# gargatik/Seamless-Through-Breaking-Rethinking-Image-Stitching-for-Optimal-Alignment

Measured on AMD Instinct MI355X. Metric: stitched image-pairs/s at 512x512, higher is better.
Workload: dtype f32 (decoder contractions, PatchEmbed's third conv and the C = 128 block tails: exact 3xbf16 split of both operands, 6 products on the bf16 matrix cores, fp32 accumulate -- error vs fp64 0.83x the fp32 MFMA chain's; everything else fp32)

## Files before the change

seamless-through-breaking-rethinking-image-stitching-for-optimal-alignment_amd/csrc/mlp_split3.h:

```cpp
#define MS3_W1_B 24576
#define MS3_W2_B 24576
#define MS3_BIAS_B 1024
#define MS3_STAGE_B (MS3_W1_B + MS3_W2_B + MS3_BIAS_B)
#define MS3_PIECES (MS3_STAGE_B / 1024)

typedef unsigned u32x4 __attribute__((ext_vector_type(4)));
typedef __bf16 bf16x2_t __attribute__((ext_vector_type(2)));
typedef float f32x2_t __attribute__((ext_vector_type(2)));

__device__ __forceinline__ unsigned ms3_pk(float a, float b) {
    const f32x2_t v = {a, b};
    return __builtin_bit_cast(unsigned, __builtin_convertvector(v, bf16x2_t));
}
__device__ __forceinline__ void ms3_split_pair(float x0, float x1, unsigned& h, unsigned& m, unsigned& l) {
    h = ms3_pk(x0, x1);
    const float r0 = x0 - __uint_as_float(h << 16), r1 = x1 - __uint_as_float(h & 0xffff0000u);
    m = ms3_pk(r0, r1);
    l = ms3_pk(r0 - __uint_as_float(m << 16), r1 - __uint_as_float(m & 0xffff0000u));
}

__global__ __launch_bounds__(256) void mlp_split3_pack_kernel(const float* __restrict__ w1, const float* __restrict__ b1, const float* __restrict__ w2,
                                                              const float* __restrict__ wp, const float* __restrict__ bp, int hidden,
                                                              unsigned char* __restrict__ image) {
    const int step = blockIdx.y, npre = wp ? 4 : 0;
    const bool pre = step < npre;
    const int c = pre ? step : step - npre;
    unsigned char* st = image + (size_t)step * MS3_STAGE_B;
    const int b = blockIdx.x, t = threadIdx.x;
    if (b < 2) {
        const int idx = b * 256 + t, r = idx >> 4, sl = idx & 15, ks = sl >> 1, lh = sl & 1;
        const float* W = (pre ? wp : w1) + (size_t)(32 * c + r) * 128;
        bf16x8 h, m, l;
#pragma unroll
        for (int e = 0; e < 8; ++e) {
            __bf16 a0, a1, a2;
            st_split3(W[16 * ks + 8 * (e >> 2) + 4 * lh + (e & 3)], a0, a1, a2);
            h[e] = a0; m[e] = a1; l[e] = a2;
        }
        unsigned char* o = st + r * 256 + ((sl ^ (r & 15)) << 4);
        *reinterpret_cast<bf16x8*>(o) = h;
        *reinterpret_cast<bf16x8*>(o + 8192) = m;
        *reinterpret_cast<bf16x8*>(o + 16384) = l;
    } else if (b < 4) {
        const int idx = (b - 2) * 256 + t, r = idx >> 2, sl = idx & 3, ks = sl >> 1, lh = sl & 1;
        bf16x8 h, m, l;
#pragma unroll
        for (int e = 0; e < 8; ++e) {
            __bf16 a0, a1, a2;
            const float v = pre ? 0.f : w2[(size_t)r * hidden + 32 * c + 16 * ks + 8 * (e >> 2) + 4 * lh + (e & 3)];
            st_split3(v, a0, a1, a2);
            h[e] = a0; m[e] = a1; l[e] = a2;
        }
        unsigned char* o = st + MS3_W1_B + r * 64 + ((sl ^ ((r >> 2) & 3)) << 4);
        *reinterpret_cast<bf16x8*>(o) = h;
        *reinterpret_cast<bf16x8*>(o + 8192) = m;
        *reinterpret_cast<bf16x8*>(o + 16384) = l;
    } else {
        float v = 0.f;
        if (t < 32) v = pre ? (bp ? bp[32 * c + t] : 0.f) : b1[32 * c + t];
        reinterpret_cast<float*>(st + MS3_W1_B + MS3_W2_B)[t] = v;
    }
}

#define MS3_SCHED_MFMA_VALU(NV)                                \
    __builtin_amdgcn_sched_group_barrier(0x008, 1, 0);         \
    __builtin_amdgcn_sched_group_barrier(0x002, NV, 0);

#define MS3_NWAVES 4

__device__ __forceinline__ float ms3_gelu(float x) {
    const float u = fabsf(x) * 0.84932180028801904272f;
    const float t = __builtin_amdgcn_rcpf(fmaf(0.2727374808792225f, u, 1.0f));
    float y = fmaf(0.5307027145f, t, -0.7265760135f);
    y = fmaf(y, t, 0.7107068705f);
    y = fmaf(y, t, -0.142248368f);
    y = fmaf(y, t, 0.127414796f);
    y = (y * t) * __builtin_amdgcn_exp2f(-(u * u));
    return fmaf(-fabsf(x), y, fmaxf(x, 0.f));
}

template <bool PROJ>
__global__ __launch_bounds__(256, 1) void rowmlp128_split3_kernel(const st_mlp_desc d, const unsigned char* __restrict__ image, const unsigned image_bytes) {
    extern __shared__ __attribute__((aligned(1024))) unsigned char sm3[];
    const int tid = threadIdx.x, lane = tid & 63, wave = __builtin_amdgcn_readfirstlane(tid >> 6);
    const int li = lane & 31, lh = lane >> 5;
    const int nblk = (d.M + 31) >> 5;
    const int G = (int)gridDim.x;
    const int blk0 = (int)blockIdx.x * MS3_NWAVES;
    const int rounds = blk0 < nblk ? (nblk - blk0 + G * MS3_NWAVES - 1) / (G * MS3_NWAVES) : 0;
    constexpr int npre = PROJ ? 4 : 0;
    const int nhc = d.hidden >> 5, spr = npre + nhc, total = rounds * spr;
    if (total == 0) return;
    const unsigned lds0 = (unsigned)(size_t)(__attribute__((address_space(3))) unsigned char*)sm3;

    int s_dma = 0, g_dma = 0, q_dma = 0;
    const unsigned vlin = (unsigned)lane << 4;
    const i32x4 rsd = make_rsrc(image, image_bytes);
    auto dma_run4 = [&](unsigned lds, unsigned soff) {
        asm volatile("s_mov_b32 m0, %0\n\ts_nop 0\n\t"
                     "buffer_load_dwordx4 %1, %2, %3 offen lds\n\t"
                     "buffer_load_dwordx4 %1, %2, %3 offen offset:1024 lds\n\t"
                     "buffer_load_dwordx4 %1, %2, %3 offen offset:2048 lds\n\t"
                     "buffer_load_dwordx4 %1, %2, %3 offen offset:3072 lds"
                     : : "s"(lds), "v"(vlin), "s"(rsd), "s"(soff) : "memory");
    };
    auto dma_run2 = [&](unsigned lds, unsigned soff) {
        asm volatile("s_mov_b32 m0, %0\n\ts_nop 0\n\t"
                     "buffer_load_dwordx4 %1, %2, %3 offen lds\n\t"
                     "buffer_load_dwordx4 %1, %2, %3 offen offset:1024 lds"
                     : : "s"(lds), "v"(vlin), "s"(rsd), "s"(soff) : "memory");
    };
    auto dma_step = [&]() {
        const unsigned dst = lds0 + (unsigned)(g_dma * MS3_STAGE_B), src = (unsigned)(s_dma * MS3_STAGE_B);
        if (PROJ && s_dma < npre) {
            const unsigned o = (unsigned)wave * 6144u;
            dma_run4(dst + o, src + o);
            dma_run2(dst + o + 4096u, src + o + 4096u);
        } else {
            const unsigned o = (unsigned)wave * 12288u;
            dma_run4(dst + o, src + o);
            dma_run4(dst + o + 4096u, src + o + 4096u);
            dma_run4(dst + o + 8192u, src + o + 8192u);
        }
        if (wave == 0) lds_dma16(rsd, dst + (unsigned)(MS3_W1_B + MS3_W2_B), vlin, src + (unsigned)(MS3_W1_B + MS3_W2_B));
        ++q_dma;
        s_dma = s_dma + 1 == spr ? 0 : s_dma + 1;
        g_dma = g_dma + 1 == 3 ? 0 : g_dma + 1;
    };
    dma_step();
    if (total > 1) dma_step();
    auto step_sync = [&]() {
        asm volatile("s_waitcnt vmcnt(0)" ::: "memory");
        __syncthreads();
        if (q_dma < total) dma_step();
    };

    int fo1[8], fo2[2];
#pragma unroll
    for (int ks = 0; ks < 8; ++ks) fo1[ks] = li * 256 + (((2 * ks + lh) ^ (li & 15)) << 4);
#pragma unroll
    for (int ks = 0; ks < 2; ++ks) fo2[ks] = MS3_W1_B + li * 64 + (((2 * ks + lh) ^ ((li >> 2) & 3)) << 4);

    u32x4 xp[3][8];
    auto split_rows = [&](const float4 (&x)[16]) {
#pragma unroll
        for (int j = 0; j < 16; ++j) {
            unsigned h0, m0, l0, h1, m1, l1;
            ms3_split_pair(x[j].x, x[j].y, h0, m0, l0);
            ms3_split_pair(x[j].z, x[j].w, h1, m1, l1);
            xp[0][j >> 1][2 * (j & 1)] = h0; xp[0][j >> 1][2 * (j & 1) + 1] = h1;
            xp[1][j >> 1][2 * (j & 1)] = m0; xp[1][j >> 1][2 * (j & 1) + 1] = m1;
            xp[2][j >> 1][2 * (j & 1)] = l0; xp[2][j >> 1][2 * (j & 1) + 1] = l1;
        }
    };
#define MS3_BF(v) __builtin_bit_cast(bf16x8, v)
#define MS3_SIX(acc, f, x0, x1, x2)                                                              \
    acc = __builtin_amdgcn_mfma_f32_32x32x16_bf16(MS3_BF(f[2]), MS3_BF(x0), acc, 0, 0, 0);       \
    acc = __builtin_amdgcn_mfma_f32_32x32x16_bf16(MS3_BF(f[0]), MS3_BF(x2), acc, 0, 0, 0);       \
    acc = __builtin_amdgcn_mfma_f32_32x32x16_bf16(MS3_BF(f[1]), MS3_BF(x1), acc, 0, 0, 0);       \
    acc = __builtin_amdgcn_mfma_f32_32x32x16_bf16(MS3_BF(f[1]), MS3_BF(x0), acc, 0, 0, 0);       \
    acc = __builtin_amdgcn_mfma_f32_32x32x16_bf16(MS3_BF(f[0]), MS3_BF(x1), acc, 0, 0, 0);       \
    acc = __builtin_amdgcn_mfma_f32_32x32x16_bf16(MS3_BF(f[0]), MS3_BF(x0), acc, 0, 0, 0);

#define MS3_CHUNK128(acc, g, DMA)                                                                                           \
    {                                                                                                                       \
        const unsigned char* ws_ = sm3 + (g) * MS3_STAGE_B;                                                                 \
        _Pragma("unroll") for (int r = 0; r < 16; ++r) acc[r] = 0.f;                                                        \
        u32x4 f[3], fn[3];                                                                                                  \
        _Pragma("unroll") for (int p = 0; p < 3; ++p) f[p] = *reinterpret_cast<const u32x4*>(ws_ + p * 8192 + fo1[0]);      \
        _Pragma("unroll") for (int ks = 0; ks < 8; ++ks) {                                                                  \
            const int kn = ks + 1 < 8 ? ks + 1 : ks;                                                                        \
            _Pragma("unroll") for (int p = 0; p < 3; ++p) fn[p] = *reinterpret_cast<const u32x4*>(ws_ + p * 8192 + fo1[kn]); \
            MS3_SIX(acc, f, xp[0][ks], xp[1][ks], xp[2][ks])                                                                \
            _Pragma("unroll") for (int p = 0; p < 3; ++p) f[p] = fn[p];                                                     \
            __builtin_amdgcn_sched_barrier(0);                                                                              \
        }                                                                                                                   \
    }
#define MS3_GELU_PAIR(ks, acc, bs)                                                                                          \
    {                                                                                                                       \
        const float2 bq = *reinterpret_cast<const float2*>(bs + 8 * ((2 * (ks)) >> 2) + 4 * lh + ((2 * (ks)) & 3));           \
        unsigned h_, m_, l_;                                                                                                \
        ms3_split_pair(ms3_gelu(acc[2 * (ks)] + bq.x), ms3_gelu(acc[2 * (ks) + 1] + bq.y), h_, m_, l_);                     \
        hp[0][(ks) >> 2][(ks) & 3] = h_; hp[1][(ks) >> 2][(ks) & 3] = m_; hp[2][(ks) >> 2][(ks) & 3] = l_;                  \
    }
#define MS3_PHASE2(wc)                                                                                                      \
    {                                                                                                                       \
        u32x4 f[3], fn[3];                                                                                                  \
        _Pragma("unroll") for (int p = 0; p < 3; ++p) f[p] = *reinterpret_cast<const u32x4*>(wc + p * 8192 + fo2[0]);       \
        _Pragma("unroll") for (int u = 0; u < 8; ++u) {                                                                     \
            const int oc = u >> 1, ks = u & 1, un = u + 1 < 8 ? u + 1 : u;                                                  \
            _Pragma("unroll") for (int p = 0; p < 3; ++p)                                                                   \
                fn[p] = *reinterpret_cast<const u32x4*>(wc + p * 8192 + (un >> 1) * 2048 + fo2[un & 1]);                    \
            MS3_SIX(o[oc], f, hp[0][ks], hp[1][ks], hp[2][ks])                                                              \
            _Pragma("unroll") for (int p = 0; p < 3; ++p) f[p] = fn[p];                                                     \
            __builtin_amdgcn_sched_barrier(0);                                                                              \
        }                                                                                                                   \
    }

    int g = 0;
    auto next_stage = [](int s) { return s + 1 == 3 ? 0 : s + 1; };
    for (int rd = 0; rd < rounds; ++rd) {
        const int blk = blk0 + wave + rd * G * MS3_NWAVES;
        if (blk >= nblk) {
            for (int s = 0; s < spr; ++s) { step_sync(); g = next_stage(g); }
            continue;
        }
        const int row = blk * 32 + li;
        const bool rok = row < d.M;
        const size_t rowc = (size_t)(rok ? row : d.M - 1);
        float4 xf[16];
#pragma unroll
        for (int j = 0; j < 16; ++j) xf[j] = *reinterpret_cast<const float4*>(d.a + rowc * d.lda + 8 * j + 4 * lh);
        if (PROJ) {
            float4 ev[16];
            if (d.res0) {
#pragma unroll
                for (int j = 0; j < 16; ++j) ev[j] = *reinterpret_cast<const float4*>(d.res0 + rowc * d.ld_res0 + 8 * j + 4 * lh);
            } else {
#pragma unroll
                for (int j = 0; j < 16; ++j) ev[j] = make_float4(0.f, 0.f, 0.f, 0.f);
            }
            split_rows(xf);
#pragma unroll
            for (int c = 0; c < 4; ++c) {
                step_sync();
                f32x16 acc;
                MS3_CHUNK128(acc, g, true)
                const float* bs = reinterpret_cast<const float*>(sm3 + g * MS3_STAGE_B + MS3_W1_B + MS3_W2_B);
#pragma unroll
                for (int jj = 0; jj < 4; ++jj) {
                    const float4 bv = *reinterpret_cast<const float4*>(bs + 8 * jj + 4 * lh);
                    const float4 e = ev[4 * c + jj];
                    xf[4 * c + jj] = make_float4((acc[4 * jj] + bv.x) + e.x, (acc[4 * jj + 1] + bv.y) + e.y, (acc[4 * jj + 2] + bv.z) + e.z, (acc[4 * jj + 3] + bv.w) + e.w);
                }
                g = next_stage(g);
            }
        }
        {
            float4 xn[16];
#pragma unroll
            for (int j = 0; j < 16; ++j) xn[j] = xf[j];
            if (d.ln) {
                float s = 0.f;
#pragma unroll
                for (int j = 0; j < 16; ++j) s += (xn[j].x + xn[j].y) + (xn[j].z + xn[j].w);
                s += __shfl_xor(s, 32, 64);
                const float mean = s * (1.0f / 128.0f);
                float v = 0.f;
#pragma unroll
                for (int j = 0; j < 16; ++j) {
                    xn[j].x -= mean; xn[j].y -= mean; xn[j].z -= mean; xn[j].w -= mean;
                    v += (xn[j].x * xn[j].x + xn[j].y * xn[j].y) + (xn[j].z * xn[j].z + xn[j].w * xn[j].w);
                }
                v += __shfl_xor(v, 32, 64);
                const float rstd = 1.0f / sqrtf(v * (1.0f / 128.0f) + d.ln_eps);
#pragma unroll
                for (int j = 0; j < 16; ++j) { xn[j].x *= rstd; xn[j].y *= rstd; xn[j].z *= rstd; xn[j].w *= rstd; }
            }
            split_rows(xn);
        }
        __builtin_amdgcn_sched_barrier(0);
        f32x16 o[4];
#pragma unroll
        for (int oc = 0; oc < 4; ++oc)
#pragma unroll
            for (int r = 0; r < 16; ++r) o[oc][r] = 0.f;
        step_sync();
        f32x16 acc;
        MS3_CHUNK128(acc, g, false)
        u32x4 hp[3][2];
#pragma unroll 1
        for (int hc = 0; hc + 1 < nhc; ++hc) {
            if (hc > 0) step_sync();
            const int gn = next_stage(g);
            const unsigned char* wc = sm3 + g * MS3_STAGE_B;
            const unsigned char* wn = sm3 + gn * MS3_STAGE_B;
            const float* bs = reinterpret_cast<const float*>(wc + MS3_W1_B + MS3_W2_B);
            f32x16 an;
#pragma unroll
            for (int r = 0; r < 16; ++r) an[r] = 0.f;
            {
                u32x4 f[3], fn[3];
#pragma unroll
                for (int p = 0; p < 3; ++p) f[p] = *reinterpret_cast<const u32x4*>(wn + p * 8192 + fo1[0]);
#pragma unroll
                for (int ks = 0; ks < 8; ++ks) {
                    const int kn = ks + 1 < 8 ? ks + 1 : ks;
#pragma unroll
                    for (int p = 0; p < 3; ++p) fn[p] = *reinterpret_cast<const u32x4*>(wn + p * 8192 + fo1[kn]);
                    MS3_SIX(an, f, xp[0][ks], xp[1][ks], xp[2][ks])
                    MS3_GELU_PAIR(ks, acc, bs)
#pragma unroll
                    for (int p = 0; p < 3; ++p) f[p] = fn[p];
                    MS3_SCHED_MFMA_VALU(7) MS3_SCHED_MFMA_VALU(7) MS3_SCHED_MFMA_VALU(7) MS3_SCHED_MFMA_VALU(7) MS3_SCHED_MFMA_VALU(7) MS3_SCHED_MFMA_VALU(7)
                    __builtin_amdgcn_sched_barrier(0);
                }
            }
            MS3_PHASE2(wc)
            acc = an;
            g = gn;
        }
        {
            if (nhc > 1) step_sync();
            const unsigned char* wc = sm3 + g * MS3_STAGE_B;
            const float* bs = reinterpret_cast<const float*>(wc + MS3_W1_B + MS3_W2_B);
#pragma unroll
            for (int ks = 0; ks < 8; ++ks) MS3_GELU_PAIR(ks, acc, bs)
            __builtin_amdgcn_sched_barrier(0);
            MS3_PHASE2(wc)
            g = next_stage(g);
        }
        if (rok) {
            const float* b2p = d.b2;
            asm volatile("" : "+s"(b2p));
#pragma unroll
            for (int oc = 0; oc < 4; ++oc) {
                float4 bb[4], e[4];
#pragma unroll
                for (int jj = 0; jj < 4; ++jj) bb[jj] = *reinterpret_cast<const float4*>(b2p + oc * 32 + 8 * jj + 4 * lh);
                if (d.res) {
#pragma unroll
                    for (int jj = 0; jj < 4; ++jj) e[jj] = *reinterpret_cast<const float4*>(d.res + rowc * d.ld_res + oc * 32 + 8 * jj + 4 * lh);
                } else {
#pragma unroll
                    for (int jj = 0; jj < 4; ++jj) e[jj] = make_float4(0.f, 0.f, 0.f, 0.f);
                }
#pragma unroll
                for (int jj = 0; jj < 4; ++jj) {
                    const int col = oc * 32 + 8 * jj + 4 * lh;
                    const float4 x = xf[4 * oc + jj];
                    float4 v = make_float4((o[oc][4 * jj] + bb[jj].x) + x.x, (o[oc][4 * jj + 1] + bb[jj].y) + x.y, (o[oc][4 * jj + 2] + bb[jj].z) + x.z,
                                           (o[oc][4 * jj + 3] + bb[jj].w) + x.w);
                    if (d.res) { v.x += e[jj].x; v.y += e[jj].y; v.z += e[jj].z; v.w += e[jj].w; }
                    *reinterpret_cast<float4*>(d.out + rowc * d.ldo + col) = v;
                }
            }
        }
    }
}

#define LS3_STAGE_B (MS3_W1_B + MS3_BIAS_B)

__global__ __launch_bounds__(256) void rowlin_split3_pack_kernel(const float* __restrict__ w, const float* __restrict__ b, unsigned char* __restrict__ image) {
    const int c = blockIdx.y, t = threadIdx.x;
    unsigned char* st = image + (size_t)c * LS3_STAGE_B;
    if (blockIdx.x < 2) {
        const int idx = blockIdx.x * 256 + t, r = idx >> 4, sl = idx & 15, ks = sl >> 1, lh = sl & 1;
        const float* W = w + (size_t)(32 * c + r) * 128;
        bf16x8 h, m, l;
#pragma unroll
        for (int e = 0; e < 8; ++e) {
            __bf16 a0, a1, a2;
            st_split3(W[16 * ks + 8 * (e >> 2) + 4 * lh + (e & 3)], a0, a1, a2);
            h[e] = a0; m[e] = a1; l[e] = a2;
        }
        unsigned char* o = st + r * 256 + ((sl ^ (r & 15)) << 4);
        *reinterpret_cast<bf16x8*>(o) = h;
        *reinterpret_cast<bf16x8*>(o + 8192) = m;
        *reinterpret_cast<bf16x8*>(o + 16384) = l;
    } else {
        reinterpret_cast<float*>(st + MS3_W1_B)[t] = (t < 32 && b) ? b[32 * c + t] : 0.f;
    }
}

template <bool AUX>
__global__ __launch_bounds__(256, 2) void rowlin128_split3_kernel(const float* __restrict__ a, const int lda, float* __restrict__ out, const int ldo, const int M,
                                                                  const int N, const int ln, const float ln_eps, const unsigned char* __restrict__ image,
                                                                  const unsigned image_bytes, const float* __restrict__ aux, const int ld_aux, const int row_div) {
    extern __shared__ __attribute__((aligned(1024))) unsigned char sm3[];
    const int tid = threadIdx.x, lane = tid & 63, wave = __builtin_amdgcn_readfirstlane(tid >> 6);
    const int li = lane & 31, lh = lane >> 5;
    const int nblk = (M + 31) >> 5;
    const int G = (int)gridDim.x;
    const int blk0 = (int)blockIdx.x * 4;
    const int rounds = blk0 < nblk ? (nblk - blk0 + G * 4 - 1) / (G * 4) : 0;
    const int spr = N >> 5, total = rounds * spr;
    if (total == 0) return;
    const unsigned lds0 = (unsigned)(size_t)(__attribute__((address_space(3))) unsigned char*)sm3;
    const i32x4 rsd = make_rsrc(image, image_bytes);
    const unsigned vlin = (unsigned)lane << 4;
    int s_dma = 0, g_dma = 0, q_dma = 0;
    auto dma_step = [&]() {
        const unsigned dst = lds0 + (unsigned)(g_dma * LS3_STAGE_B), src = (unsigned)(s_dma * LS3_STAGE_B), o = (unsigned)wave * 6144u;
        asm volatile("s_mov_b32 m0, %0\n\ts_nop 0\n\t"
                     "buffer_load_dwordx4 %1, %2, %3 offen lds\n\t"
                     "buffer_load_dwordx4 %1, %2, %3 offen offset:1024 lds\n\t"
                     "buffer_load_dwordx4 %1, %2, %3 offen offset:2048 lds\n\t"
                     "buffer_load_dwordx4 %1, %2, %3 offen offset:3072 lds"
                     : : "s"(dst + o), "v"(vlin), "s"(rsd), "s"(src + o) : "memory");
        asm volatile("s_mov_b32 m0, %0\n\ts_nop 0\n\t"
                     "buffer_load_dwordx4 %1, %2, %3 offen lds\n\t"
                     "buffer_load_dwordx4 %1, %2, %3 offen offset:1024 lds"
                     : : "s"(dst + o + 4096u), "v"(vlin), "s"(rsd), "s"(src + o + 4096u) : "memory");
        if (wave == 0) lds_dma16(rsd, dst + (unsigned)MS3_W1_B, vlin, src + (unsigned)MS3_W1_B);
        ++q_dma;
        s_dma = s_dma + 1 == spr ? 0 : s_dma + 1;
        g_dma = g_dma + 1 == 3 ? 0 : g_dma + 1;
    };
    dma_step();
    if (total > 1) dma_step();
    int fo1[8];
#pragma unroll
    for (int ks = 0; ks < 8; ++ks) fo1[ks] = li * 256 + (((2 * ks + lh) ^ (li & 15)) << 4);
    int g = 0;
    for (int rd = 0; rd < rounds; ++rd) {
        const int blk = blk0 + wave + rd * G * 4;
        const bool active = blk < nblk;
        const int row = blk * 32 + li;
        const bool rok = active && row < M;
        const size_t rowc = (size_t)(active && row < M ? row : M - 1);
        u32x4 xp[3][8];
        if (active) {
            float4 x[16];
#pragma unroll
            for (int j = 0; j < 16; ++j) x[j] = *reinterpret_cast<const float4*>(a + rowc * lda + 8 * j + 4 * lh);
            if (ln) {
                float s = 0.f;
#pragma unroll
                for (int j = 0; j < 16; ++j) s += (x[j].x + x[j].y) + (x[j].z + x[j].w);
                s += __shfl_xor(s, 32, 64);
                const float mean = s * (1.0f / 128.0f);
                float v = 0.f;
#pragma unroll
                for (int j = 0; j < 16; ++j) {
                    x[j].x -= mean; x[j].y -= mean; x[j].z -= mean; x[j].w -= mean;
                    v += (x[j].x * x[j].x + x[j].y * x[j].y) + (x[j].z * x[j].z + x[j].w * x[j].w);
                }
                v += __shfl_xor(v, 32, 64);
                const float rstd = 1.0f / sqrtf(v * (1.0f / 128.0f) + ln_eps);
#pragma unroll
                for (int j = 0; j < 16; ++j) { x[j].x *= rstd; x[j].y *= rstd; x[j].z *= rstd; x[j].w *= rstd; }
            }
#pragma unroll
            for (int j = 0; j < 16; ++j) {
                unsigned h0, m0, l0, h1, m1, l1;
                ms3_split_pair(x[j].x, x[j].y, h0, m0, l0);
                ms3_split_pair(x[j].z, x[j].w, h1, m1, l1);
                xp[0][j >> 1][2 * (j & 1)] = h0; xp[0][j >> 1][2 * (j & 1) + 1] = h1;
                xp[1][j >> 1][2 * (j & 1)] = m0; xp[1][j >> 1][2 * (j & 1) + 1] = m1;
                xp[2][j >> 1][2 * (j & 1)] = l0; xp[2][j >> 1][2 * (j & 1) + 1] = l1;
            }
        }
        __builtin_amdgcn_sched_barrier(0);
#pragma unroll 1
        for (int c = 0; c < spr; ++c) {
            if (c > 0 && active) asm volatile("s_waitcnt vmcnt(4)" ::: "memory");
            else asm volatile("s_waitcnt vmcnt(0)" ::: "memory");
            __syncthreads();
            if (q_dma < total) dma_step();
            if (active) {
                const unsigned char* ws_ = sm3 + g * LS3_STAGE_B;
                float4 ev[4];
                if (AUX) {
#pragma unroll
                    for (int jj = 0; jj < 4; ++jj) ev[jj] = *reinterpret_cast<const float4*>(aux + (rowc / (size_t)row_div) * ld_aux + (c << 5) + 8 * jj + 4 * lh);
                }
                f32x16 acc;
#pragma unroll
                for (int r = 0; r < 16; ++r) acc[r] = 0.f;
                u32x4 f[3], fn[3];
#pragma unroll
                for (int p = 0; p < 3; ++p) f[p] = *reinterpret_cast<const u32x4*>(ws_ + p * 8192 + fo1[0]);
#pragma unroll
                for (int ks = 0; ks < 8; ++ks) {
                    const int kn = ks + 1 < 8 ? ks + 1 : ks;
#pragma unroll
                    for (int p = 0; p < 3; ++p) fn[p] = *reinterpret_cast<const u32x4*>(ws_ + p * 8192 + fo1[kn]);
                    MS3_SIX(acc, f, xp[0][ks], xp[1][ks], xp[2][ks])
#pragma unroll
                    for (int p = 0; p < 3; ++p) f[p] = fn[p];
                    __builtin_amdgcn_sched_barrier(0);
                }
                const float* bs = reinterpret_cast<const float*>(ws_ + MS3_W1_B);
                float4 v[4];
#pragma unroll
                for (int jj = 0; jj < 4; ++jj) {
                    const float4 bv = *reinterpret_cast<const float4*>(bs + 8 * jj + 4 * lh);
                    v[jj] = make_float4(acc[4 * jj] + bv.x, acc[4 * jj + 1] + bv.y, acc[4 * jj + 2] + bv.z, acc[4 * jj + 3] + bv.w);
                    if (AUX) { v[jj].x += ev[jj].x; v[jj].y += ev[jj].y; v[jj].z += ev[jj].z; v[jj].w += ev[jj].w; }
                }
                if (rok) {
#pragma unroll
                    for (int jj = 0; jj < 4; ++jj) *reinterpret_cast<float4*>(out + rowc * ldo + (c << 5) + 8 * jj + 4 * lh) = v[jj];
                }
            }
            g = g + 1 == 3 ? 0 : g + 1;
        }
    }
}


#define PT3_W1_B 12288
#define PT3_IMAGE_B (4 * PT3_W1_B + 4 * MS3_W2_B)
#define PT3_VEC_B 1536

__global__ __launch_bounds__(256) void pe_tail_split3_pack_kernel(const float* __restrict__ w1, const int ld1, const float* __restrict__ w2, unsigned char* __restrict__ image) {
    const int c = blockIdx.y, t = threadIdx.x;
    bf16x8 h, m, l;
    unsigned char* o;
    if (blockIdx.x == 0) {
        const int r = t >> 3, sl = t & 7, ks = sl >> 1, lh = sl & 1;
#pragma unroll
        for (int e = 0; e < 8; ++e) {
            __bf16 a0, a1, a2;
            st_split3(w1[(size_t)(32 * c + r) * ld1 + 16 * ks + 8 * (e >> 2) + 4 * lh + (e & 3)], a0, a1, a2);
            h[e] = a0; m[e] = a1; l[e] = a2;
        }
        o = image + c * PT3_W1_B + r * 128 + ((sl ^ ((r >> 1) & 7)) << 4);
        *reinterpret_cast<bf16x8*>(o) = h;
        *reinterpret_cast<bf16x8*>(o + 4096) = m;
        *reinterpret_cast<bf16x8*>(o + 8192) = l;
    } else {
        const int idx = (blockIdx.x - 1) * 256 + t, r = idx >> 2, sl = idx & 3, ks = sl >> 1, lh = sl & 1;
#pragma unroll
        for (int e = 0; e < 8; ++e) {
            __bf16 a0, a1, a2;
            st_split3(w2[(size_t)r * 128 + 32 * c + 16 * ks + 8 * (e >> 2) + 4 * lh + (e & 3)], a0, a1, a2);
            h[e] = a0; m[e] = a1; l[e] = a2;
        }
        o = image + 4 * PT3_W1_B + c * MS3_W2_B + r * 64 + ((sl ^ ((r >> 2) & 3)) << 4);
        *reinterpret_cast<bf16x8*>(o) = h;
        *reinterpret_cast<bf16x8*>(o + 8192) = m;
        *reinterpret_cast<bf16x8*>(o + 16384) = l;
    }
}

template <bool TABINV>
__global__ __launch_bounds__(256, 1) void pe_tail_split3_kernel(const float* __restrict__ x, const float* __restrict__ tab, const unsigned char* __restrict__ image,
                                                                const float* __restrict__ b2, const float* __restrict__ gamma, const float* __restrict__ beta,
                                                                const float eps, float* __restrict__ out, const int R, const int P) {
    extern __shared__ __attribute__((aligned(1024))) unsigned char sm3[];
    const int tid = threadIdx.x, lane = tid & 63, wave = __builtin_amdgcn_readfirstlane(tid >> 6);
    const int li = lane & 31, lh = lane >> 5;
    const unsigned lds0 = (unsigned)(size_t)(__attribute__((address_space(3))) unsigned char*)sm3;
    {
        const i32x4 rsd = make_rsrc(image, (unsigned)PT3_IMAGE_B);
        const unsigned vlin = (unsigned)lane << 4;
#pragma unroll
        for (int u = 0; u < 9; ++u) {
            const unsigned o = (unsigned)wave * 36864u + (unsigned)u * 4096u;
            asm volatile("s_mov_b32 m0, %0\n\ts_nop 0\n\t"
                         "buffer_load_dwordx4 %1, %2, %3 offen lds\n\t"
                         "buffer_load_dwordx4 %1, %2, %3 offen offset:1024 lds\n\t"
                         "buffer_load_dwordx4 %1, %2, %3 offen offset:2048 lds\n\t"
                         "buffer_load_dwordx4 %1, %2, %3 offen offset:3072 lds"
                         : : "s"(lds0 + o), "v"(vlin), "s"(rsd), "s"(o) : "memory");
        }
        float* vec = reinterpret_cast<float*>(sm3 + PT3_IMAGE_B);
        if (tid < 128) { vec[tid] = b2[tid]; vec[128 + tid] = gamma[tid]; vec[256 + tid] = beta[tid]; }
        asm volatile("s_waitcnt vmcnt(0)" ::: "memory");
        __syncthreads();
    }
    const float* vec = reinterpret_cast<const float*>(sm3 + PT3_IMAGE_B) + 4 * lh;
    const int fo1_row = li * 128, fo1_x = (li >> 1) & 7;
    int fo2[2];
#pragma unroll
    for (int ks = 0; ks < 2; ++ks) fo2[ks] = 4 * PT3_W1_B + li * 64 + (((2 * ks + lh) ^ ((li >> 2) & 3)) << 4);
    const int nblk = (R + 31) >> 5, stride = (int)gridDim.x * 4;
    int blk = (int)blockIdx.x * 4 + wave;
    if (blk >= nblk) return;

    float4 xa[8], tv[16];
    auto load_rows = [&](int b, float4 (&xo)[8]) {
        const int row = b * 32 + li;
        const float* xr = x + (size_t)(row < R ? row : R - 1) * 64 + 4 * lh;
#pragma unroll
        for (int j = 0; j < 8; ++j) xo[j] = *reinterpret_cast<const float4*>(xr + 8 * j);
    };
    auto load_table = [&](int b, float4 (&to)[16]) {
        const int row = b * 32 + li;
        const float* tr = tab + (size_t)(row % P) * 128 + 4 * lh;
#pragma unroll
        for (int j = 0; j < 16; ++j) to[j] = *reinterpret_cast<const float4*>(tr + 8 * j);
    };
    load_rows(blk, xa);
    load_table(blk, tv);
#define PT3_BF(v) __builtin_bit_cast(bf16x8, v)
#pragma unroll 1
    for (; blk < nblk; blk += stride) {
        const int row = blk * 32 + li;
        const bool rok = row < R;
        const size_t rowc = (size_t)(rok ? row : R - 1);
        u32x4 xp[3][4];
#pragma unroll
        for (int j = 0; j < 8; ++j) {
            unsigned h0, m0, l0, h1, m1, l1;
            ms3_split_pair(xa[j].x, xa[j].y, h0, m0, l0);
            ms3_split_pair(xa[j].z, xa[j].w, h1, m1, l1);
            xp[0][j >> 1][2 * (j & 1)] = h0; xp[0][j >> 1][2 * (j & 1) + 1] = h1;
            xp[1][j >> 1][2 * (j & 1)] = m0; xp[1][j >> 1][2 * (j & 1) + 1] = m1;
            xp[2][j >> 1][2 * (j & 1)] = l0; xp[2][j >> 1][2 * (j & 1) + 1] = l1;
        }
        float4 tc[16];
#pragma unroll
        for (int j = 0; j < 16; ++j) tc[j] = tv[j];
        const int nb = blk + stride;
        load_rows(nb < nblk ? nb : blk, xa);
        if (!TABINV) load_table(nb < nblk ? nb : blk, tv);
        __builtin_amdgcn_sched_barrier(0);
        f32x16 o[4];
#pragma unroll
        for (int oc = 0; oc < 4; ++oc)
#pragma unroll
            for (int r = 0; r < 16; ++r) o[oc][r] = 0.f;
        f32x16 acc;
#pragma unroll
        for (int r = 0; r < 16; ++r) acc[r] = 0.f;
        {
            const unsigned char* w1 = sm3 + fo1_row;
            u32x4 f[3], fn[3];
#pragma unroll
            for (int p = 0; p < 3; ++p) f[p] = *reinterpret_cast<const u32x4*>(w1 + p * 4096 + (((0 + lh) ^ fo1_x) << 4));
#pragma unroll
            for (int ks = 0; ks < 4; ++ks) {
                const int kn = ks + 1 < 4 ? ks + 1 : ks;
#pragma unroll
                for (int p = 0; p < 3; ++p) fn[p] = *reinterpret_cast<const u32x4*>(w1 + p * 4096 + (((2 * kn + lh) ^ fo1_x) << 4));
                MS3_SIX(acc, f, xp[0][ks], xp[1][ks], xp[2][ks])
#pragma unroll
                for (int p = 0; p < 3; ++p) f[p] = fn[p];
                __builtin_amdgcn_sched_barrier(0);
            }
        }
        __builtin_amdgcn_sched_barrier(0);
#pragma unroll
        for (int c = 0; c < 4; ++c) {
            u32x4 hp[3][2];
            f32x16 an;
#pragma unroll
            for (int r = 0; r < 16; ++r) an[r] = 0.f;
            u32x4 g1[3], g1n[3];
            if (c < 3) {
#pragma unroll
                for (int p = 0; p < 3; ++p) g1[p] = *reinterpret_cast<const u32x4*>(sm3 + (c + 1) * PT3_W1_B + fo1_row + p * 4096 + (((0 + lh) ^ fo1_x) << 4));
            }
#pragma unroll
            for (int ks = 0; ks < 4; ++ks) {
                if (c < 3) {
                    const unsigned char* w1 = sm3 + (c + 1) * PT3_W1_B + fo1_row;
                    const int kn = ks + 1 < 4 ? ks + 1 : ks;
#pragma unroll
                    for (int p = 0; p < 3; ++p) g1n[p] = *reinterpret_cast<const u32x4*>(w1 + p * 4096 + (((2 * kn + lh) ^ fo1_x) << 4));
                    MS3_SIX(an, g1, xp[0][ks], xp[1][ks], xp[2][ks])
#pragma unroll
                    for (int p = 0; p < 3; ++p) g1[p] = g1n[p];
                }
                {
                    const float4 t4 = tc[4 * c + ks];
                    unsigned h0, m0, l0, h1, m1, l1;
                    ms3_split_pair(fmaxf(acc[4 * ks] + t4.x, 0.f), fmaxf(acc[4 * ks + 1] + t4.y, 0.f), h0, m0, l0);
                    ms3_split_pair(fmaxf(acc[4 * ks + 2] + t4.z, 0.f), fmaxf(acc[4 * ks + 3] + t4.w, 0.f), h1, m1, l1);
                    hp[0][ks >> 1][2 * (ks & 1)] = h0; hp[0][ks >> 1][2 * (ks & 1) + 1] = h1;
                    hp[1][ks >> 1][2 * (ks & 1)] = m0; hp[1][ks >> 1][2 * (ks & 1) + 1] = m1;
                    hp[2][ks >> 1][2 * (ks & 1)] = l0; hp[2][ks >> 1][2 * (ks & 1) + 1] = l1;
                }
                if (c < 3) { MS3_SCHED_MFMA_VALU(5) MS3_SCHED_MFMA_VALU(5) MS3_SCHED_MFMA_VALU(5) MS3_SCHED_MFMA_VALU(5) MS3_SCHED_MFMA_VALU(5) MS3_SCHED_MFMA_VALU(5) }
                __builtin_amdgcn_sched_barrier(0);
            }
            {
                const unsigned char* wc = sm3 + c * MS3_W2_B;
                u32x4 f[3], fn[3];
#pragma unroll
                for (int p = 0; p < 3; ++p) f[p] = *reinterpret_cast<const u32x4*>(wc + p * 8192 + fo2[0]);
#pragma unroll
                for (int u = 0; u < 8; ++u) {
                    const int oc = u >> 1, ks = u & 1, un = u + 1 < 8 ? u + 1 : u;
#pragma unroll
                    for (int p = 0; p < 3; ++p) fn[p] = *reinterpret_cast<const u32x4*>(wc + p * 8192 + (un >> 1) * 2048 + fo2[un & 1]);
                    MS3_SIX(o[oc], f, hp[0][ks], hp[1][ks], hp[2][ks])
#pragma unroll
                    for (int p = 0; p < 3; ++p) f[p] = fn[p];
                    __builtin_amdgcn_sched_barrier(0);
                }
            }
            acc = an;
        }
        float s = 0.f;
#pragma unroll
        for (int oc = 0; oc < 4; ++oc)
#pragma unroll
            for (int jj = 0; jj < 4; ++jj) {
                const float4 bb = *reinterpret_cast<const float4*>(vec + oc * 32 + 8 * jj);
                o[oc][4 * jj] += bb.x; o[oc][4 * jj + 1] += bb.y; o[oc][4 * jj + 2] += bb.z; o[oc][4 * jj + 3] += bb.w;
                s += (o[oc][4 * jj] + o[oc][4 * jj + 1]) + (o[oc][4 * jj + 2] + o[oc][4 * jj + 3]);
            }
        s += __shfl_xor(s, 32, 64);
        const float mean = s * (1.0f / 128.0f);
        float v = 0.f;
#pragma unroll
        for (int oc = 0; oc < 4; ++oc)
#pragma unroll
            for (int r = 0; r < 16; ++r) { o[oc][r] -= mean; v += o[oc][r] * o[oc][r]; }
        v += __shfl_xor(v, 32, 64);
        const float rstd = 1.0f / sqrtf(v * (1.0f / 128.0f) + eps);
        if (rok) {
#pragma unroll
            for (int oc = 0; oc < 4; ++oc)
#pragma unroll
                for (int jj = 0; jj < 4; ++jj) {
                    const float4 gg = *reinterpret_cast<const float4*>(vec + 128 + oc * 32 + 8 * jj), be = *reinterpret_cast<const float4*>(vec + 256 + oc * 32 + 8 * jj);
                    *reinterpret_cast<float4*>(out + rowc * 128 + oc * 32 + 8 * jj + 4 * lh) =
                        make_float4(o[oc][4 * jj] * rstd * gg.x + be.x, o[oc][4 * jj + 1] * rstd * gg.y + be.y, o[oc][4 * jj + 2] * rstd * gg.z + be.z,
                                    o[oc][4 * jj + 3] * rstd * gg.w + be.w);
                }
        }
    }
#undef PT3_BF
}

#undef MS3_PHASE2
#undef MS3_GELU_PAIR
#undef MS3_CHUNK128
#undef MS3_SIX
#undef MS3_BF
```

Before: 92.69.

## Software-pipeline MLP fc2 of previous chunk with fc1 of next chunk

Restructures the row-MLP hidden-chunk loop so the second matmul (fc2) for chunk h-1 is interleaved with the first matmul (fc1) for chunk h+1 and the GELU of chunk h, instead of running fc2 as a separate phase after each fc1. The LDS weight DMA is split into independent W1 and W2 streams issued by different waves, so W2 for a stage can be fetched one step later than W1. The aim is a denser mix of MFMA and VALU work and fewer exposed phase boundaries, at the cost of more live registers (hq, extra accumulators and fragments) and more complex stage-buffer lifetime logic.

Result: no change. 93.10 (median of 6 runs) (+0.4%).

```diff
diff --git a/seamless-through-breaking-rethinking-image-stitching-for-optimal-alignment_amd/csrc/mlp_split3.h b/seamless-through-breaking-rethinking-image-stitching-for-optimal-alignment_amd/csrc/mlp_split3.h
--- a/seamless-through-breaking-rethinking-image-stitching-for-optimal-alignment_amd/csrc/mlp_split3.h
+++ b/seamless-through-breaking-rethinking-image-stitching-for-optimal-alignment_amd/csrc/mlp_split3.h
@@ -93,7 +93,7 @@
     if (total == 0) return;
     const unsigned lds0 = (unsigned)(size_t)(__attribute__((address_space(3))) unsigned char*)sm3;
 
-    int s_dma = 0, g_dma = 0, q_dma = 0;
+    int s1 = 0, g1 = 0, n1 = 0, s2 = 0, g2 = 0, n2 = 0;
     const unsigned vlin = (unsigned)lane << 4;
     const i32x4 rsd = make_rsrc(image, image_bytes);
     auto dma_run4 = [&](unsigned lds, unsigned soff) {
@@ -104,35 +104,39 @@
                      "buffer_load_dwordx4 %1, %2, %3 offen offset:3072 lds"
                      : : "s"(lds), "v"(vlin), "s"(rsd), "s"(soff) : "memory");
     };
-    auto dma_run2 = [&](unsigned lds, unsigned soff) {
-        asm volatile("s_mov_b32 m0, %0\n\ts_nop 0\n\t"
-                     "buffer_load_dwordx4 %1, %2, %3 offen lds\n\t"
-                     "buffer_load_dwordx4 %1, %2, %3 offen offset:1024 lds"
-                     : : "s"(lds), "v"(vlin), "s"(rsd), "s"(soff) : "memory");
-    };
-    auto dma_step = [&]() {
-        const unsigned dst = lds0 + (unsigned)(g_dma * MS3_STAGE_B), src = (unsigned)(s_dma * MS3_STAGE_B);
-        if (PROJ && s_dma < npre) {
-            const unsigned o = (unsigned)wave * 6144u;
-            dma_run4(dst + o, src + o);
-            dma_run2(dst + o + 4096u, src + o + 4096u);
-        } else {
+    auto dma_run12 = [&](unsigned lds, unsigned soff) {
+        dma_run4(lds, soff);
+        dma_run4(lds + 4096u, soff + 4096u);
+        dma_run4(lds + 8192u, soff + 8192u);
+    };
+    auto dma_w1 = [&]() {
+        if (wave < 2) {
             const unsigned o = (unsigned)wave * 12288u;
-            dma_run4(dst + o, src + o);
-            dma_run4(dst + o + 4096u, src + o + 4096u);
-            dma_run4(dst + o + 8192u, src + o + 8192u);
-        }
-        if (wave == 0) lds_dma16(rsd, dst + (unsigned)(MS3_W1_B + MS3_W2_B), vlin, src + (unsigned)(MS3_W1_B + MS3_W2_B));
-        ++q_dma;
-        s_dma = s_dma + 1 == spr ? 0 : s_dma + 1;
-        g_dma = g_dma + 1 == 3 ? 0 : g_dma + 1;
-    };
-    dma_step();
-    if (total > 1) dma_step();
+            dma_run12(lds0 + (unsigned)(g1 * MS3_STAGE_B) + o, (unsigned)(s1 * MS3_STAGE_B) + o);
+        }
+        ++n1;
+        s1 = s1 + 1 == spr ? 0 : s1 + 1;
+        g1 = g1 + 1 == 3 ? 0 : g1 + 1;
+    };
+    auto dma_w2 = [&]() {
+        const unsigned dst = lds0 + (unsigned)(g2 * MS3_STAGE_B), src = (unsigned)(s2 * MS3_STAGE_B);
+        if (wave >= 2 && !(PROJ && s2 < npre)) {
+            const unsigned o = (unsigned)MS3_W1_B + (unsigned)(wave - 2) * 12288u;
+            dma_run12(dst + o, src + o);
+        }
+        if (wave == 3) lds_dma16(rsd, dst + (unsigned)(MS3_W1_B + MS3_W2_B), vlin, src + (unsigned)(MS3_W1_B + MS3_W2_B));
+        ++n2;
+        s2 = s2 + 1 == spr ? 0 : s2 + 1;
+        g2 = g2 + 1 == 3 ? 0 : g2 + 1;
+    };
+    dma_w1();
+    dma_w2();
+    if (total > 1) dma_w1();
     auto step_sync = [&]() {
         asm volatile("s_waitcnt vmcnt(0)" ::: "memory");
         __syncthreads();
-        if (q_dma < total) dma_step();
+        if (n1 < total) dma_w1();
+        if (n2 < total) dma_w2();
     };
 
     int fo1[8], fo2[2];
@@ -196,6 +200,37 @@
             __builtin_amdgcn_sched_barrier(0);                                                                              \
         }                                                                                                                   \
     }
+#define MS3_PIPE_STEP(FC1, FC2, wn, wq, ws)                                                                                 \
+    {                                                                                                                       \
+        const float* bs = reinterpret_cast<const float*>((ws) + MS3_W1_B + MS3_W2_B);                                       \
+        u32x4 f[3], fn[3], e[3], en[3];                                                                                     \
+        if (FC1) { _Pragma("unroll") for (int p = 0; p < 3; ++p) f[p] = *reinterpret_cast<const u32x4*>((wn) + p * 8192 + fo1[0]); } \
+        if (FC2) { _Pragma("unroll") for (int p = 0; p < 3; ++p) e[p] = *reinterpret_cast<const u32x4*>((wq) + p * 8192 + fo2[0]); } \
+        _Pragma("unroll") for (int ks = 0; ks < 8; ++ks) {                                                                  \
+            const int kn = ks + 1 < 8 ? ks + 1 : ks;                                                                        \
+            if (FC1) {                                                                                                      \
+                _Pragma("unroll") for (int p = 0; p < 3; ++p) fn[p] = *reinterpret_cast<const u32x4*>((wn) + p * 8192 + fo1[kn]); \
+                MS3_SIX(an, f, xp[0][ks], xp[1][ks], xp[2][ks])                                                             \
+            }                                                                                                               \
+            if (FC2) {                                                                                                      \
+                _Pragma("unroll") for (int p = 0; p < 3; ++p)                                                               \
+                    en[p] = *reinterpret_cast<const u32x4*>((wq) + p * 8192 + (kn >> 1) * 2048 + fo2[kn & 1]);              \
+                MS3_SIX(o[ks >> 1], e, hq[0][ks & 1], hq[1][ks & 1], hq[2][ks & 1])                                         \
+            }                                                                                                               \
+            MS3_GELU_PAIR(ks, acc, bs)                                                                                      \
+            if (FC1) { _Pragma("unroll") for (int p = 0; p < 3; ++p) f[p] = fn[p]; }                                        \
+            if (FC2) { _Pragma("unroll") for (int p = 0; p < 3; ++p) e[p] = en[p]; }                                        \
+            if (FC1 && FC2) {                                                                                               \
+                MS3_SCHED_MFMA_VALU(3) MS3_SCHED_MFMA_VALU(4) MS3_SCHED_MFMA_VALU(3) MS3_SCHED_MFMA_VALU(4)                 \
+                MS3_SCHED_MFMA_VALU(3) MS3_SCHED_MFMA_VALU(4) MS3_SCHED_MFMA_VALU(3) MS3_SCHED_MFMA_VALU(4)                 \
+                MS3_SCHED_MFMA_VALU(3) MS3_SCHED_MFMA_VALU(4) MS3_SCHED_MFMA_VALU(3) MS3_SCHED_MFMA_VALU(4)                 \
+            } else if (FC1 || FC2) {                                                                                        \
+                MS3_SCHED_MFMA_VALU(7) MS3_SCHED_MFMA_VALU(7) MS3_SCHED_MFMA_VALU(7)                                        \
+                MS3_SCHED_MFMA_VALU(7) MS3_SCHED_MFMA_VALU(7) MS3_SCHED_MFMA_VALU(7)                                        \
+            }                                                                                                               \
+            __builtin_amdgcn_sched_barrier(0);                                                                              \
+        }                                                                                                                   \
+    }
 
     int g = 0;
     auto next_stage = [](int s) { return s + 1 == 3 ? 0 : s + 1; };
@@ -266,50 +301,35 @@
 #pragma unroll
             for (int r = 0; r < 16; ++r) o[oc][r] = 0.f;
         step_sync();
-        f32x16 acc;
+        f32x16 acc, an;
         MS3_CHUNK128(acc, g, false)
-        u32x4 hp[3][2];
+        u32x4 hp[3][2], hq[3][2];
+        if (nhc > 1) {
+            int gq = g, gn = next_stage(g);
+#pragma unroll
+            for (int r = 0; r < 16; ++r) an[r] = 0.f;
+            MS3_PIPE_STEP(true, false, sm3 + gn * MS3_STAGE_B, sm3, sm3 + g * MS3_STAGE_B)
+            acc = an; gq = g; g = gn;
 #pragma unroll 1
-        for (int hc = 0; hc + 1 < nhc; ++hc) {
-            if (hc > 0) step_sync();
-            const int gn = next_stage(g);
-            const unsigned char* wc = sm3 + g * MS3_STAGE_B;
-            const unsigned char* wn = sm3 + gn * MS3_STAGE_B;
-            const float* bs = reinterpret_cast<const float*>(wc + MS3_W1_B + MS3_W2_B);
-            f32x16 an;
-#pragma unroll
-            for (int r = 0; r < 16; ++r) an[r] = 0.f;
-            {
-                u32x4 f[3], fn[3];
-#pragma unroll
-                for (int p = 0; p < 3; ++p) f[p] = *reinterpret_cast<const u32x4*>(wn + p * 8192 + fo1[0]);
-#pragma unroll
-                for (int ks = 0; ks < 8; ++ks) {
-                    const int kn = ks + 1 < 8 ? ks + 1 : ks;
-#pragma unroll
-                    for (int p = 0; p < 3; ++p) fn[p] = *reinterpret_cast<const u32x4*>(wn + p * 8192 + fo1[kn]);
-                    MS3_SIX(an, f, xp[0][ks], xp[1][ks], xp[2][ks])
-                    MS3_GELU_PAIR(ks, acc, bs)
-#pragma unroll
-                    for (int p = 0; p < 3; ++p) f[p] = fn[p];
-                    MS3_SCHED_MFMA_VALU(7) MS3_SCHED_MFMA_VALU(7) MS3_SCHED_MFMA_VALU(7) MS3_SCHED_MFMA_VALU(7) MS3_SCHED_MFMA_VALU(7) MS3_SCHED_MFMA_VALU(7)
-                    __builtin_amdgcn_sched_barrier(0);
-                }
-            }
-            MS3_PHASE2(wc)
-            acc = an;
-            g = gn;
-        }
-        {
-            if (nhc > 1) step_sync();
-            const unsigned char* wc = sm3 + g * MS3_STAGE_B;
-            const float* bs = reinterpret_cast<const float*>(wc + MS3_W1_B + MS3_W2_B);
-#pragma unroll
-            for (int ks = 0; ks < 8; ++ks) MS3_GELU_PAIR(ks, acc, bs)
-            __builtin_amdgcn_sched_barrier(0);
-            MS3_PHASE2(wc)
-            g = next_stage(g);
-        }
+            for (int hc = 1; hc + 1 < nhc; ++hc) {
+#pragma unroll
+                for (int p = 0; p < 3; ++p) { hq[p][0] = hp[p][0]; hq[p][1] = hp[p][1]; }
+                step_sync();
+                gn = next_stage(g);
+#pragma unroll
+                for (int r = 0; r < 16; ++r) an[r] = 0.f;
+                MS3_PIPE_STEP(true, true, sm3 + gn * MS3_STAGE_B, sm3 + gq * MS3_STAGE_B, sm3 + g * MS3_STAGE_B)
+                acc = an; gq = g; g = gn;
+            }
+#pragma unroll
+            for (int p = 0; p < 3; ++p) { hq[p][0] = hp[p][0]; hq[p][1] = hp[p][1]; }
+            step_sync();
+            MS3_PIPE_STEP(false, true, sm3, sm3 + gq * MS3_STAGE_B, sm3 + g * MS3_STAGE_B)
+        } else {
+            MS3_PIPE_STEP(false, false, sm3, sm3, sm3 + g * MS3_STAGE_B)
+        }
+        MS3_PHASE2(sm3 + g * MS3_STAGE_B)
+        g = next_stage(g);
         if (rok) {
             const float* b2p = d.b2;
             asm volatile("" : "+s"(b2p));
@@ -708,6 +728,7 @@
 #undef PT3_BF
 }
 
+#undef MS3_PIPE_STEP
 #undef MS3_PHASE2
 #undef MS3_GELU_PAIR
 #undef MS3_CHUNK128
```
